# liyi14/mx-DeepIM

Measured on NVIDIA B200. Metric: 480x640 4-iter pose refinements/sec, higher is better.
Workload: dtype fp16

## Files before the change

### mx-deepim_b200/csrc/conv_igemm.cuh

```cuda
#pragma once
#include <cuda.h>
#include <cuda_fp16.h>
#include "common.cuh"

namespace dim {

struct ConvKParams {
  CUtensorMap a_map[4];
  CUtensorMap a_lo_map[4];
  CUtensorMap b_map;
  CUtensorMap b_lo_map;
  CUtensorMap b2_map;
  CUtensorMap b2_lo_map;
  int KH, KW, stride, cchunks;
  int BW, BH, n_col_tiles;
  int Hq, Ho, Wo, Bn;
  int out_Hp, out_Wp, out_py, out_px, Cout;
  int kblocks, ksplit;
  int f16;
  uint32_t idesc;
  float slope;
  const float *bias;
  __nv_bfloat16 *out_hi, *out_lo;
  float *partial;
  int in_off_r, in_off_c;
  int out_sy, out_sx, out_oy, out_ox, out_H, out_W, out_cs, out_coff;
  struct PixBuf { const __nv_bfloat16 *p; int Hp, Wp, py, px, cs, coff; } addend, mask;
  int mask_climit;
};

namespace ptx {

__device__ __forceinline__ uint32_t smem_u32(const void *p) { return (uint32_t)__cvta_generic_to_shared(p); }

__device__ __forceinline__ bool elect_one() {
  uint32_t pred;
  asm volatile(
      "{\n\t.reg .pred p;\n\telect.sync _|p, 0xFFFFFFFF;\n\tselp.u32 %0, 1, 0, p;\n\t}"
      : "=r"(pred));
  return pred != 0;
}

// ... 128 lines not shown
  d |= (uint64_t)((saddr & 0x3FFFFu) >> 4);
  d |= (uint64_t)1 << 16;
  d |= (uint64_t)((sbo_bytes >> 4) & 0x3FFFu) << 32;
  d |= (uint64_t)1 << 46;
  d |= (uint64_t)layout_type << 61;
  return d;
}

}

__device__ __forceinline__ void sts128(uint32_t addr, uint4 v) {
  asm volatile("st.shared.v4.b32 [%0], {%1, %2, %3, %4};" ::"r"(addr), "r"(v.x), "r"(v.y), "r"(v.z), "r"(v.w) : "memory");
}
__device__ __forceinline__ uint4 lds128(uint32_t addr) {
  uint4 v;
  asm volatile("ld.shared.v4.b32 {%0, %1, %2, %3}, [%4];" : "=r"(v.x), "=r"(v.y), "=r"(v.z), "=r"(v.w) : "r"(addr) : "memory");
  return v;
}
__device__ __forceinline__ float4 lds128f(uint32_t addr) {
  float4 v;
  asm volatile("ld.shared.v4.f32 {%0, %1, %2, %3}, [%4];" : "=f"(v.x), "=f"(v.y), "=f"(v.z), "=f"(v.w) : "r"(addr));
  return v;
}

__device__ __forceinline__ uint32_t pack2_f16(float a, float b) {
  uint32_t r;
  asm("cvt.rn.satfinite.f16x2.f32 %0, %1, %2;" : "=r"(r) : "f"(b), "f"(a));
  return r;
}
__device__ __forceinline__ uint32_t pack2_bf16(float a, float b) {
  uint32_t r;
  asm("cvt.rn.bf16x2.f32 %0, %1, %2;" : "=r"(r) : "f"(b), "f"(a));
  return r;
}

template <bool SPLIT3>
__device__ __forceinline__ void epilogue_store64(const uint32_t *r, const float *bias_s, float slope, uint8_t *stage,
                                                 __nv_bfloat16 *out_hi, __nv_bfloat16 *out_lo, long long my_off,
                                                 bool my_valid, int lane, bool f16 = false) {
  __align__(16) uint32_t h[32];
  __align__(16) uint32_t l[SPLIT3 ? 32 : 4];
  const uint32_t ba = ptx::smem_u32(bias_s), sa = ptx::smem_u32(stage);
#pragma unroll
  for (int j = 0; j < 64; j += 4) {
    const float4 b4 = lds128f(ba + j * 4);
    float v0 = __uint_as_float(r[j]) + b4.x, v1 = __uint_as_float(r[j + 1]) + b4.y;
    float v2 = __uint_as_float(r[j + 2]) + b4.z, v3 = __uint_as_float(r[j + 3]) + b4.w;
    v0 = v0 > 0.f ? v0 : v0 * slope;
    v1 = v1 > 0.f ? v1 : v1 * slope;
    v2 = v2 > 0.f ? v2 : v2 * slope;
    v3 = v3 > 0.f ? v3 : v3 * slope;
    if (!SPLIT3 && f16) {
      h[j >> 1] = pack2_f16(v0, v1);
      h[(j >> 1) + 1] = pack2_f16(v2, v3);
    } else {
      const uint32_t h0 = pack2_bf16(v0, v1), h1 = pack2_bf16(v2, v3);
      h[j >> 1] = h0;
      h[(j >> 1) + 1] = h1;
      if (SPLIT3) {
        l[j >> 1] = pack2_bf16(v0 - __uint_as_float(h0 << 16), v1 - __uint_as_float(h0 & 0xFFFF0000u));
        l[(j >> 1) + 1] = pack2_bf16(v2 - __uint_as_float(h1 << 16), v3 - __uint_as_float(h1 & 0xFFFF0000u));
      }
    }
  }
  const unsigned vmask = __ballot_sync(0xffffffffu, my_valid);
  const int ch = lane & 7;
#pragma unroll
  for (int pass = 0; pass < (SPLIT3 ? 2 : 1); ++pass) {
    const uint32_t *src = pass ? l : h;
    __nv_bfloat16 *out = pass ? out_lo : out_hi;
#pragma unroll
    for (int c = 0; c < 8; ++c)
      sts128(sa + lane * 128 + ((c ^ (lane & 7)) << 4), *reinterpret_cast<const uint4 *>(src + c * 4));
    __syncwarp();
#pragma unroll
    for (int i = 0; i < 8; ++i) {
      const int row = i * 4 + (lane >> 3);
      const long long off = __shfl_sync(0xffffffffu, my_off, row);
      const uint4 v = lds128(sa + row * 128 + ((ch ^ (row & 7)) << 4));
      if ((vmask >> row) & 1u) *reinterpret_cast<uint4 *>(out + off + ch * 8) = v;
    }
    __syncwarp();
  }
}

template <bool SPLIT3, bool LINEAR = false, bool BIAS_REG = false>
__device__ __forceinline__ void epilogue_store32(const uint32_t *r, const float *bias_s, float slope, uint8_t *stage,
                                                 __nv_bfloat16 *out_hi, __nv_bfloat16 *out_lo, long long my_off,
                                                 bool my_valid, int lane, bool f16, int n_valid = 32, int row_stride = 0) {
  __align__(16) uint32_t h[16];
  __align__(16) uint32_t l[SPLIT3 ? 16 : 4];
  const uint32_t ba = BIAS_REG ? 0u : ptx::smem_u32(bias_s), sa = ptx::smem_u32(stage);
#pragma unroll
  for (int j = 0; j < 32; j += 4) {
    const float4 b4 = BIAS_REG ? make_float4(bias_s[j], bias_s[j + 1], bias_s[j + 2], bias_s[j + 3]) : lds128f(ba + j * 4);
    float v0 = __uint_as_float(r[j]) + b4.x, v1 = __uint_as_float(r[j + 1]) + b4.y;
    float v2 = __uint_as_float(r[j + 2]) + b4.z, v3 = __uint_as_float(r[j + 3]) + b4.w;
    v0 = v0 > 0.f ? v0 : v0 * slope;
    v1 = v1 > 0.f ? v1 : v1 * slope;
    v2 = v2 > 0.f ? v2 : v2 * slope;
    v3 = v3 > 0.f ? v3 : v3 * slope;
    if (!SPLIT3 && f16) {
      h[j >> 1] = pack2_f16(v0, v1);
      h[(j >> 1) + 1] = pack2_f16(v2, v3);
    } else {
      const uint32_t h0 = pack2_bf16(v0, v1), h1 = pack2_bf16(v2, v3);
      h[j >> 1] = h0;
      h[(j >> 1) + 1] = h1;
      if (SPLIT3) {
        l[j >> 1] = pack2_bf16(v0 - __uint_as_float(h0 << 16), v1 - __uint_as_float(h0 & 0xFFFF0000u));
        l[(j >> 1) + 1] = pack2_bf16(v2 - __uint_as_float(h1 << 16), v3 - __uint_as_float(h1 & 0xFFFF0000u));
      }
    }
  }
  const unsigned vmask = LINEAR ? 0u : __ballot_sync(0xffffffffu, my_valid);
  const int ch = lane & 3;
#pragma unroll
  for (int pass = 0; pass < (SPLIT3 ? 2 : 1); ++pass) {
    const uint32_t *src = pass ? l : h;
    __nv_bfloat16 *out = pass ? out_lo : out_hi;
#pragma unroll
    for (int c = 0; c < 4; ++c)
      sts128(sa + lane * 64 + ((c ^ ((lane >> 1) & 3)) << 4), *reinterpret_cast<const uint4 *>(src + c * 4));
    __syncwarp();
#pragma unroll
    for (int i = 0; i < 4; ++i) {
      const int row = i * 8 + (lane >> 2);
      const uint4 v = lds128(sa + row * 64 + ((ch ^ ((row >> 1) & 3)) << 4));
      if (LINEAR) {
        if (row < n_valid) *reinterpret_cast<uint4 *>(out + my_off + (long long)row * row_stride + ch * 8) = v;
      } else {
        const long long off = __shfl_sync(0xffffffffu, my_off, row);
        if ((vmask >> row) & 1u) *reinterpret_cast<uint4 *>(out + off + ch * 8) = v;
      }
    }
    __syncwarp();
  }
// ... 42 lines not shown
    const int row = i * 4 + (lane >> 3);
    const long long off = __shfl_sync(0xffffffffu, my_off, row);
    const uint4 v = lds128(sa + row * 128 + ((ch ^ (row & 7)) << 4));
    if ((vmask >> row) & 1u) *reinterpret_cast<uint4 *>(p.out_hi + off + ch * 8) = v;
  }
  __syncwarp();
}

template <int BLOCK_N, int BLOCK_K, int STAGES, bool SPLIT3, bool RESIDENT_B, int KBLOCKS_RES>
struct ConvSmem2 {
  static constexpr int A_BYTES = 128 * BLOCK_K * 2;
  static constexpr int B_BYTES = BLOCK_N * BLOCK_K * 2;
  static constexpr int NPREC = SPLIT3 ? 2 : 1;
  static constexpr int STAGE_BYTES = (A_BYTES + (RESIDENT_B ? 0 : B_BYTES)) * NPREC;
  static constexpr int RES_BYTES = RESIDENT_B ? KBLOCKS_RES * B_BYTES * NPREC : 0;
  static constexpr int EPI_BYTES = 4 * 4096 + 4096 ;
  static constexpr int TOTAL = STAGES * STAGE_BYTES + RES_BYTES + EPI_BYTES + 1024  + 512 ;
};

__device__ __forceinline__ void mbar_arrive(uint64_t *bar) {
  asm volatile("mbarrier.arrive.shared::cta.b64 _, [%0];" ::"r"(ptx::smem_u32(bar)) : "memory");
}

template <int BLOCK_N, int BLOCK_K, int STAGES, bool SPLIT3, bool RESIDENT_B, int KBLOCKS_RES, int EPI = 0>
__global__ void __launch_bounds__(192) conv_igemm_persistent_kernel(const __grid_constant__ ConvKParams p,
                                                                    const int total_tiles, const int n_tiles) {
  using S = ConvSmem2<BLOCK_N, BLOCK_K, STAGES, SPLIT3, RESIDENT_B, KBLOCKS_RES>;
  constexpr uint32_t LAYOUT = (BLOCK_K == 64) ? 2u : 4u;
  constexpr uint32_t SBO = 8u * BLOCK_K * 2u;
  constexpr uint32_t ACC_COLS = BLOCK_N < 32 ? 32 : BLOCK_N;
  constexpr uint32_t TMEM_COLS = 2 * ACC_COLS;

  extern __shared__ uint8_t smem_raw[];
  uint8_t *smem = reinterpret_cast<uint8_t *>((reinterpret_cast<uintptr_t>(smem_raw) + 1023) & ~(uintptr_t)1023);
  uint8_t *res = smem + STAGES * S::STAGE_BYTES;
  uint8_t *epi = res + S::RES_BYTES;
  float *bias_s = reinterpret_cast<float *>(epi + 4 * 4096);
  uint64_t *full_bar = reinterpret_cast<uint64_t *>(epi + S::EPI_BYTES);
  uint64_t *empty_bar = full_bar + STAGES;
  uint64_t *tmem_full_bar = empty_bar + STAGES;
  uint64_t *tmem_empty_bar = tmem_full_bar + 2;
  uint64_t *res_bar = tmem_empty_bar + 2;
  uint32_t *tmem_slot = reinterpret_cast<uint32_t *>(res_bar + 1);

  const int warp = threadIdx.x >> 5, lane = threadIdx.x & 31;
  const int kb0 = 0, kb1 = p.kblocks;

  if (warp == 0 && lane == 0) {
    for (int s = 0; s < STAGES; ++s) {
      ptx::mbar_init(&full_bar[s], 1);
      ptx::mbar_init(&empty_bar[s], 1);
    }
    for (int a = 0; a < 2; ++a) {
      ptx::mbar_init(&tmem_full_bar[a], 1);
      ptx::mbar_init(&tmem_empty_bar[a], 4);
    }
    ptx::mbar_init(res_bar, 1);
    ptx::fence_barrier_init();
    ptx::prefetch_tmap(&p.b_map);
    ptx::prefetch_tmap(&p.a_map[0]);
  }
  for (int c = threadIdx.x; c < p.Cout && c < 1024; c += blockDim.x) bias_s[c] = p.bias ? p.bias[c] : 0.f;
  if (warp == 1) ptx::tmem_alloc(tmem_slot, TMEM_COLS);
  ptx::tc_fence_before();
  __syncthreads();
  ptx::tc_fence_after();
  const uint32_t tmem_base = *tmem_slot;

  if (warp == 0) {
    {
      if (RESIDENT_B) {
        ptx::mbar_expect_tx(res_bar, (uint32_t)S::RES_BYTES);
        for (int kb = 0; kb < KBLOCKS_RES; ++kb) {
          ptx::tma_load_2d(res + kb * S::B_BYTES, &p.b_map, res_bar, kb * BLOCK_K, 0);
          if (SPLIT3) ptx::tma_load_2d(res + (KBLOCKS_RES + kb) * S::B_BYTES, &p.b_lo_map, res_bar, kb * BLOCK_K, 0);
        }
      }
      const uint32_t tx = (uint32_t)(p.BW * p.BH * BLOCK_K * 2 + (RESIDENT_B ? 0 : BLOCK_N * BLOCK_K * 2)) * S::NPREC;
      int s = 0;
      uint32_t ph = 0;
      for (int tile = blockIdx.x; tile < total_tiles; tile += gridDim.x) {
        const int nt = tile % n_tiles, mt = tile / n_tiles;
        const int col_tile = mt % p.n_col_tiles, row_tile = mt / p.n_col_tiles;
        const int g0 = row_tile * p.BH, ow0 = col_tile * p.BW, n0 = nt * BLOCK_N;
        for (int kb = kb0; kb < kb1; ++kb) {
          ptx::mbar_wait(&empty_bar[s], ph ^ 1u);
          const int tap = kb / p.cchunks, cc = kb - tap * p.cchunks;
          const int kh = tap / p.KW, kw = tap - kh * p.KW;
          int view = 0, dr = kh, dc = kw;
          if (p.stride == 2) {
            view = ((kh & 1) << 1) | (kw & 1);
            dr = kh >> 1;
            dc = kw >> 1;
          }
          uint8_t *st = smem + s * S::STAGE_BYTES;
          if (EPI) { dr += p.in_off_r; dc += p.in_off_c; }
          if (ptx::elect_one()) {
            ptx::mbar_expect_tx_raw(&full_bar[s], tx);
            ptx::tma_load_3d_raw(st, &p.a_map[view], &full_bar[s], cc * BLOCK_K, ow0 + dc, g0 + dr);
            uint8_t *nxt = st + S::A_BYTES;
            if (!RESIDENT_B) {
              ptx::tma_load_2d_raw(nxt, &p.b_map, &full_bar[s], kb * BLOCK_K, n0);
              nxt += S::B_BYTES;
            }
            if (SPLIT3) {
              ptx::tma_load_3d_raw(nxt, &p.a_lo_map[view], &full_bar[s], cc * BLOCK_K, ow0 + dc, g0 + dr);
              if (!RESIDENT_B) ptx::tma_load_2d_raw(nxt + S::A_BYTES, &p.b_lo_map, &full_bar[s], kb * BLOCK_K, n0);
            }
          }
          __syncwarp();
          if (++s == STAGES) { s = 0; ph ^= 1u; }
        }
      }
    }
  } else if (warp == 1) {
    {
      if (RESIDENT_B) {
        ptx::mbar_wait(res_bar, 0);
        ptx::tc_fence_after();
      }
      int s = 0, as = 0;
      uint32_t ph = 0, aph = 0;
      for (int tile = blockIdx.x; tile < total_tiles; tile += gridDim.x) {
        ptx::mbar_wait(&tmem_empty_bar[as], aph ^ 1u);
        ptx::tc_fence_after();
        const uint32_t tmem_acc = tmem_base + (uint32_t)as * ACC_COLS;
        for (int kb = kb0; kb < kb1; ++kb) {
          ptx::mbar_wait(&full_bar[s], ph);
          ptx::tc_fence_after();
          const uint32_t a_hi = ptx::smem_u32(smem + s * S::STAGE_BYTES);
          uint32_t b_hi, a_lo, b_lo;
          if (RESIDENT_B) {
            b_hi = ptx::smem_u32(res + kb * S::B_BYTES);
            b_lo = ptx::smem_u32(res + (KBLOCKS_RES + kb) * S::B_BYTES);
            a_lo = a_hi + S::A_BYTES;
          } else {
            b_hi = a_hi + S::A_BYTES;
            a_lo = b_hi + S::B_BYTES;
            b_lo = a_lo + S::A_BYTES;
          }
          if (ptx::elect_one()) {
            const uint64_t da0 = ptx::umma_desc(a_hi, SBO, LAYOUT), db0 = ptx::umma_desc(b_hi, SBO, LAYOUT);
            const uint64_t dal0 = ptx::umma_desc(a_lo, SBO, LAYOUT), dbl0 = ptx::umma_desc(b_lo, SBO, LAYOUT);
#pragma unroll
            for (int k = 0; k < BLOCK_K / 16; ++k) {
              const uint32_t acc = (kb > kb0 || k > 0) ? 1u : 0u;
              const uint64_t da = da0 + (uint64_t)(2 * k), db = db0 + (uint64_t)(2 * k);
              ptx::umma_f16_raw(tmem_acc, da, db, p.idesc, acc);
              if (SPLIT3) {
                ptx::umma_f16_raw(tmem_acc, dal0 + (uint64_t)(2 * k), db, p.idesc, 1u);
                ptx::umma_f16_raw(tmem_acc, da, dbl0 + (uint64_t)(2 * k), p.idesc, 1u);
              }
            }
            ptx::umma_commit_raw(&empty_bar[s]);
          }
          __syncwarp();
          if (++s == STAGES) { s = 0; ph ^= 1u; }
        }
        ptx::umma_commit(&tmem_full_bar[as]);
        if (++as == 2) { as = 0; aph ^= 1u; }
      }
    }
  } else {
    const int quad = warp & 3;
    const int m = quad * 32 + lane;
    const int bh = m / p.BW, bw = m - bh * p.BW;
    uint8_t *stg = epi + (warp - 2) * 4096;
    int as = 0;
    uint32_t aph = 0;
    for (int tile = blockIdx.x; tile < total_tiles; tile += gridDim.x) {
      ptx::mbar_wait(&tmem_full_bar[as], aph);
      ptx::tc_fence_after();
      const uint32_t trow = tmem_base + ((uint32_t)(quad * 32) << 16) + (uint32_t)as * ACC_COLS;
      if (EPI == 1) {
        const int nt = tile % n_tiles, mt = tile / n_tiles;
        const int col_tile = mt % p.n_col_tiles, row_tile = mt / p.n_col_tiles;
        const int g = row_tile * p.BH + bh, ow = col_tile * p.BW + bw, n0 = nt * BLOCK_N;
        const int n_img = g / p.Hq, oh = g - n_img * p.Hq;
        const int y = oh * p.out_sy + p.out_oy, x = ow * p.out_sx + p.out_ox;
        const bool valid = (m < p.BW * p.BH) && (n_img < p.Bn) && (oh < p.Ho) && (ow < p.Wo) && y >= 0 && y < p.out_H &&
                           x >= 0 && x < p.out_W;
        const long long my_off =
            (((long long)n_img * p.out_Hp + y + p.out_py) * p.out_Wp + x + p.out_px) * p.out_cs + p.out_coff + n0;
        const long long add_off =
            (((long long)n_img * p.addend.Hp + y + p.addend.py) * p.addend.Wp + x + p.addend.px) * p.addend.cs + p.addend.coff + n0;
        const long long mask_off =
            (((long long)n_img * p.mask.Hp + y + p.mask.py) * p.mask.Wp + x + p.mask.px) * p.mask.cs + p.mask.coff + n0;
#pragma unroll 1
        for (int c = 0; c < BLOCK_N; c += 64) {
          uint32_t r[64];
          ptx::tmem_ld_32x32(trow + c, r);
          ptx::tmem_ld_32x32(trow + c + 32, r + 32);
          if (c + 64 >= BLOCK_N) {
            ptx::tc_fence_before();
            __syncwarp();
            if (lane == 0) mbar_arrive(&tmem_empty_bar[as]);
          }
          epilogue_generic64(r, p, bias_s + ((n0 + c) & 1023), stg, my_off + c, add_off + c, mask_off + c, valid,
                             n0 + c < p.mask_climit, n0 + c < p.Cout, lane);
        }
      } else {
        const int nt = tile % n_tiles, mt = tile / n_tiles;
        const int col_tile = mt % p.n_col_tiles, row_tile = mt / p.n_col_tiles;
        const int g = row_tile * p.BH + bh, ow = col_tile * p.BW + bw, n0 = nt * BLOCK_N;
        const int n_img = g / p.Hq, oh = g - n_img * p.Hq;
        const bool valid = (m < p.BW * p.BH) && (n_img < p.Bn) && (oh < p.Ho) && (ow < p.Wo);
        const long long my_off =
            (((long long)n_img * p.out_Hp + oh + p.out_py) * p.out_Wp + ow + p.out_px) * p.Cout + n0;
#pragma unroll 1
        for (int c = 0; c < BLOCK_N; c += 64) {
          uint32_t r[64];
          ptx::tmem_ld_32x32(trow + c, r);
          ptx::tmem_ld_32x32(trow + c + 32, r + 32);
          if (c + 64 >= BLOCK_N) {
            ptx::tc_fence_before();
            __syncwarp();
            if (lane == 0) mbar_arrive(&tmem_empty_bar[as]);
          }
          epilogue_store64<SPLIT3>(r, bias_s + n0 + c, p.slope, stg, p.out_hi, p.out_lo, my_off + c, valid, lane, p.f16 != 0);
        }
      }
      if (++as == 2) { as = 0; aph ^= 1u; }
    }
  }
  ptx::tc_fence_before();
  __syncthreads();
  if (warp == 1) {
    ptx::tc_fence_after();
    ptx::tmem_dealloc(tmem_base, TMEM_COLS);
  }
}

__device__ __forceinline__ void tma_load_4d(void *dst, const CUtensorMap *map, uint64_t *bar, int c0, int c1, int c2,
                                            int c3) {
  if (ptx::elect_one())
  asm volatile(
      "cp.async.bulk.tensor.4d.shared::cluster.global.mbarrier::complete_tx::bytes [%0], [%1, {%3, %4, %5, %6}], [%2];" ::
          "r"(ptx::smem_u32(dst)),
      "l"((uint64_t)map), "r"(ptx::smem_u32(bar)), "r"(c0), "r"(c1), "r"(c2), "r"(c3)
      : "memory");
}
__device__ __forceinline__ uint64_t umma_desc_interleave(uint32_t saddr, uint32_t lbo_bytes, uint32_t sbo_bytes) {
// ... 137 lines not shown
    const int quad = warp & 3, set = (warp - 2) >> 2;
    uint8_t *stg = epi + (warp - 2) * STG;
    const int as = set;
    uint32_t aph = 0;
    const int n_cols_valid = min(p.BW, p.Wo - ow0) - quad * 32;
    for (int t = set; t < n_rows; t += 2) {
      const int g = g_lo + t;
      const int n_img = g / p.Hq, oh = g - n_img * p.Hq;
      const bool row_ok = (n_img < p.Bn) && (oh < p.Ho);
      ptx::mbar_wait(&tmem_full_bar[as], aph);
      ptx::tc_fence_after();
      const uint32_t trow = tmem_base + ((uint32_t)(quad * 32) << 16) + (uint32_t)as * ACC_COLS;
      const long long warp_off =
          (((long long)n_img * p.out_Hp + oh + p.out_py) * p.out_Wp + (ow0 + quad * 32) + p.out_px) * 64;
      uint32_t r[64];
      ptx::tmem_ld_32x32(trow, r);
      ptx::tmem_ld_32x32(trow + 32, r + 32);
      ptx::tc_fence_before();
      __syncwarp();
      if (lane == 0) mbar_arrive(&tmem_empty_bar[as]);
#pragma unroll
      for (int half = 0; half < 2; ++half)
        epilogue_store32<SPLIT3, true>(r + half * 32, bias_s + half * 32, p.slope, stg, p.out_hi, p.out_lo, warp_off + half * 32,
                                             true, lane, p.f16 != 0, row_ok ? n_cols_valid : 0, 64);
      aph ^= 1u;
    }
  }
  ptx::tc_fence_before();
  __syncthreads();
  if (warp == 1) {
    ptx::tc_fence_after();
    ptx::tmem_dealloc(tmem_base, TMEM_COLS);
  }
}

template <int STAGES>
__global__ void __launch_bounds__(320) conv1_stack_kernel(const __grid_constant__ ConvKParams p, const int rows_total,
                                                          const int rows_per_chunk, const int chunks_per_col,
                                                          const int strip_bytes ) {
  constexpr uint32_t TMEM_COLS = 512;
  constexpr int B_BYTES = 64 * 32 * 2 , DW_BYTES = 4 * B_BYTES, RES_BYTES = 4 * DW_BYTES;
  constexpr int EPI_BYTES = 8 * 2048 + 256;
  extern __shared__ uint8_t smem_raw[];
  uint8_t *smem = reinterpret_cast<uint8_t *>((reinterpret_cast<uintptr_t>(smem_raw) + 511) & ~(uintptr_t)511);
  uint8_t *res = smem;
  uint8_t *ring = smem + RES_BYTES;
  uint8_t *epi = ring + STAGES * strip_bytes;
// ... 123 lines not shown
      const bool mine = v >= 3;
      int n_img = 0, oh = 0;
      if (mine) { n_img = g / p.Hq; oh = g - n_img * p.Hq; }
      const bool row_ok = mine && (n_img < p.Bn) && (oh < p.Ho);
      ptx::mbar_wait(&acc_full_bar[v & 7], ((uint32_t)(v >> 3)) & 1u);
      ptx::tc_fence_after();
      const uint32_t tcol = tmem_base + ((uint32_t)(quad * 32) << 16) + (uint32_t)((v & 7) * 64);
      uint32_t r[64];
      if (row_ok) {
        ptx::tmem_ld_32x32(tcol, r);
        ptx::tmem_ld_32x32(tcol + 32, r + 32);
      }
      ptx::tmem_zero_32x32(tcol);
      ptx::tmem_zero_32x32(tcol + 32);
      ptx::tc_fence_before();
      __syncwarp();
      if (lane == 0) mbar_arrive(&acc_empty_bar[v & 7]);
      if (row_ok) {
        const long long warp_off =
            (((long long)n_img * p.out_Hp + oh + p.out_py) * p.out_Wp + (ow0 + quad * 32) + p.out_px) * 64;
#pragma unroll
        for (int half = 0; half < 2; ++half)
          epilogue_store32<false, true, true>(r + half * 32, breg + half * 32, p.slope, stg, p.out_hi, p.out_lo, warp_off + half * 32,
                                              true, lane, p.f16 != 0, n_cols_valid, 64);
      }
    }
  }
  ptx::tc_fence_before();
  __syncthreads();
  if (warp == 1) {
    ptx::tc_fence_after();
    ptx::tmem_dealloc(tmem_base, TMEM_COLS);
  }
}

namespace ptx2 {
__device__ __forceinline__ uint32_t cluster_ctarank() {
  uint32_t r;
  asm volatile("mov.u32 %0, %%cluster_ctarank;" : "=r"(r));
  return r;
}
__device__ __forceinline__ void cluster_sync() {
  asm volatile("barrier.cluster.arrive.release.aligned;\n\tbarrier.cluster.wait.acquire.aligned;" ::: "memory");
}
constexpr uint32_t kPeerBitMask = 0xFEFFFFFFu;
__device__ __forceinline__ void tma_load_3d(void *dst, const CUtensorMap *map, uint64_t *bar, int c0, int c1, int c2) {
  if (ptx::elect_one())
// ... 203 lines not shown
          ptx::tmem_ld_32x32(trow + c, r);
          if (valid) {
#pragma unroll
            for (int j = 0; j < 32; j += 4)
              *reinterpret_cast<uint4 *>(dst + c + j) = make_uint4(r[j], r[j + 1], r[j + 2], r[j + 3]);
          }
        }
        ptx::tc_fence_before();
        __syncwarp();
        if (lane == 0) ptx2::mbar_arrive_leader(&tmem_empty_bar[as]);
      } else {
        const long long my_off =
            (((long long)n_img * p.out_Hp + oh + p.out_py) * p.out_Wp + ow + p.out_px) * p.Cout + n0;
#pragma unroll 1
        for (int c = 0; c < BLOCK_N; c += 64) {
          uint32_t r[64];
          ptx::tmem_ld_32x32(trow + c, r);
          ptx::tmem_ld_32x32(trow + c + 32, r + 32);
          if (c + 64 >= BLOCK_N) {
            ptx::tc_fence_before();
            __syncwarp();
            if (lane == 0) ptx2::mbar_arrive_leader(&tmem_empty_bar[as]);
          }
          epilogue_store64<SPLIT3>(r, bias_s + n0 + c, p.slope, stg, p.out_hi, p.out_lo, my_off + c, valid, lane, p.f16 != 0);
        }
      }
      if (++as == 2) { as = 0; aph ^= 1u; }
    }
  }
  ptx::tc_fence_before();
  __syncthreads();
  ptx2::cluster_sync();
  if (warp == 1) {
    ptx::tc_fence_after();
    ptx2::tmem_dealloc(tmem_base, TMEM_COLS);
  }
}

static __global__ void __launch_bounds__(256) conv_splitk_finalize_kernel(const float *partial, int ksplit, int npix,
                                                                   int Cout, int Ho, int Wo, int out_Hp, int out_Wp,
                                                                   int out_py, int out_px, const float *bias,
                                                                   float slope, __nv_bfloat16 *out_hi,
                                                                   __nv_bfloat16 *out_lo, int f16) {
  const size_t idx4 = ((size_t)blockIdx.x * blockDim.x + threadIdx.x) * 4;
  if (idx4 >= (size_t)npix * Cout) return;
  const size_t opix = idx4 / Cout;
  const int c = (int)(idx4 - opix * Cout);
// ... 26 lines not shown
```

### mx-deepim_b200/csrc/net.cu

```cuda
#include <cuda_fp16.h>
#include <string.h>

#include <mutex>

#include "net_state.cuh"

namespace dim {

static void build_geometry(NetState *ns, int H, int W) {
  int h = H, w = W;
  for (int i = 0; i < 10; ++i) {
    const LayerSpec &s = kLayers[i];
    LayerGeom &g = ns->g[i];
    g.Cin = s.Cin; g.Cout = s.Cout; g.k = s.k; g.stride = s.stride; g.pad = s.pad;
    g.Hin = h; g.Win = w;
    g.Ho = (h + 2 * s.pad - s.k) / s.stride + 1;
    g.Wo = (w + 2 * s.pad - s.k) / s.stride + 1;
    if (g.Ho < 1) g.Ho = 1;
    if (g.Wo < 1) g.Wo = 1;
    int Hp = h + 2 * s.pad, Wp = w + 2 * s.pad;
    if (s.stride == 2) { Hp += Hp & 1; Wp += Wp & 1; }
    g.py = g.px = s.pad;
    if (i == 0) {
      g.rows = Hp / 2; g.cols = Wp / 2; g.Cbuf = 32;
// ... 131 lines not shown
      const uint64_t str[1] = {Ktot * 2};
      const uint32_t box[2] = {(uint32_t)g.BLOCK_K, (uint32_t)g.BLOCK_N};
      __nv_bfloat16 *wop = f16 ? ns->w_f16[i] : ns->w_hi[i];
      if (int rc = encode_map(&kp.b_map, wop, 2, dims, str, box, g.BLOCK_K)) return rc;
      if (int rc = encode_map(&kp.b_lo_map, ns->w_lo[i], 2, dims, str, box, g.BLOCK_K)) return rc;
      const uint32_t box2[2] = {(uint32_t)g.BLOCK_K, (uint32_t)(g.BLOCK_N / 2)};
      if (int rc = encode_map(&kp.b2_map, wop, 2, dims, str, box2, g.BLOCK_K)) return rc;
      if (int rc = encode_map(&kp.b2_lo_map, ns->w_lo[i], 2, dims, str, box2, g.BLOCK_K)) return rc;
    }
    kp.KH = g.KH; kp.KW = g.KW; kp.stride = g.stride_eff; kp.cchunks = g.Ceff / g.BLOCK_K;
    kp.BW = g.BW; kp.BH = g.BH; kp.n_col_tiles = g.n_col_tiles;
    kp.Hq = g.Hq; kp.Ho = g.Ho; kp.Wo = g.Wo; kp.Bn = B;
    if (i < 9) {
      const LayerGeom &nx = ns->g[i + 1];
      kp.out_Hp = nx.rows; kp.out_Wp = nx.cols; kp.out_py = nx.py; kp.out_px = nx.px;
    } else {
      kp.out_Hp = g.Ho; kp.out_Wp = g.Wo; kp.out_py = 0; kp.out_px = 0;
    }
    kp.Cout = g.Cout;
    kp.kblocks = g.kblocks;
    kp.ksplit = tm.ksplit[i] = choose_ksplit(ns, g, B);
    kp.idesc = make_idesc(g.pair ? 256 : 128, g.BLOCK_N, f16);
    kp.f16 = f16 ? 1 : 0;
    kp.slope = 0.1f;
    kp.bias = ns->bias[i];
    kp.out_hi = ns->act_hi[i + 1];
    kp.out_lo = ns->act_lo[i + 1];
    kp.partial = ns->conv_partial;
  }
  return 0;
}

template <bool F16>
__device__ __forceinline__ void mma_bf16_16816(float *c, const uint32_t *a, uint32_t b0, uint32_t b1) {
  if (F16)
    asm volatile(
        "mma.sync.aligned.m16n8k16.row.col.f32.f16.f16.f32 {%0,%1,%2,%3}, {%4,%5,%6,%7}, {%8,%9}, {%0,%1,%2,%3};"
        : "+f"(c[0]), "+f"(c[1]), "+f"(c[2]), "+f"(c[3])
        : "r"(a[0]), "r"(a[1]), "r"(a[2]), "r"(a[3]), "r"(b0), "r"(b1));
  else
    asm volatile(
        "mma.sync.aligned.m16n8k16.row.col.f32.bf16.bf16.f32 {%0,%1,%2,%3}, {%4,%5,%6,%7}, {%8,%9}, {%0,%1,%2,%3};"
        : "+f"(c[0]), "+f"(c[1]), "+f"(c[2]), "+f"(c[3])
        : "r"(a[0]), "r"(a[1]), "r"(a[2]), "r"(a[3]), "r"(b0), "r"(b1));
}

// ... 258 lines not shown
    for (int o = 0; o < 256; ++o)
      for (int c = 0; c < 1024; ++c)
        for (int hw = 0; hw < 80; ++hw) p[(size_t)o * FC6_K + (size_t)hw * 1024 + c] = W[10][(size_t)o * FC6_K + (size_t)c * 80 + hw];
    std::vector<__nv_bfloat16> hb, lb, fb;
    split_bf16(p.data(), p.size(), hb, lb, fb);
    if (int rc = upload(ctx, &ns->fc6_w_hi, hb)) return rc;
    if (int rc = upload(ctx, &ns->fc6_w_lo, lb)) return rc;
    if (int rc = upload(ctx, &ns->fc6_w_f16, fb)) return rc;
    if (int rc = upload(ctx, &ns->fc6_b, std::vector<float>(Bv[10], Bv[10] + 256))) return rc;
    std::vector<float> t((size_t)256 * 256);
    for (int o = 0; o < 256; ++o)
      for (int k = 0; k < 256; ++k) t[(size_t)k * 256 + o] = W[11][(size_t)o * 256 + k];
    if (int rc = upload(ctx, &ns->fc7_wT, t)) return rc;
    if (int rc = upload(ctx, &ns->fc7_b, std::vector<float>(Bv[11], Bv[11] + 256))) return rc;
    if (int rc = upload(ctx, &ns->rot_w, std::vector<float>(W[12], W[12] + 4 * 256))) return rc;
    if (int rc = upload(ctx, &ns->rot_b, std::vector<float>(Bv[12], Bv[12] + 4))) return rc;
    if (int rc = upload(ctx, &ns->trans_w, std::vector<float>(W[13], W[13] + 3 * 256))) return rc;
    if (int rc = upload(ctx, &ns->trans_b, std::vector<float>(Bv[13], Bv[13] + 3))) return rc;
  }
  ns->loaded = true;
  return 0;
}

template <int BN, int BK, int ST, bool S3, bool RES, int KRES>
static int launch_conv2(NetState *ns, const ConvKParams &kp, int total_tiles, int n_tiles, int cap, cudaStream_t st) {
  using S = ConvSmem2<BN, BK, ST, S3, RES, KRES>;
  static bool attr_set = false;
  if (!attr_set) {
    DIM_CHECK(cudaFuncSetAttribute(conv_igemm_persistent_kernel<BN, BK, ST, S3, RES, KRES>,
                                   cudaFuncAttributeMaxDynamicSharedMemorySize, S::TOTAL));
    attr_set = true;
  }
  const int grid = total_tiles < cap ? total_tiles : cap;
  conv_igemm_persistent_kernel<BN, BK, ST, S3, RES, KRES><<<grid, 192, S::TOTAL, st>>>(kp, total_tiles, n_tiles);
  DIM_LAUNCH_CHECK();
  return 0;
}

template <int BN, int ST, bool S3>
static int launch_pair(const ConvKParams &kp, int pair_tiles, int n_tiles, int sms, cudaStream_t st) {
  using S = ConvSmemPair<BN, ST, S3>;
  static bool attr_set = false;
  if (!attr_set) {
    DIM_CHECK(cudaFuncSetAttribute(conv_igemm_pair_kernel<BN, ST, S3>, cudaFuncAttributeMaxDynamicSharedMemorySize,
                                   S::TOTAL));
    attr_set = true;
  }
  const int pairs = pair_tiles < sms / 2 ? pair_tiles : sms / 2;
  conv_igemm_pair_kernel<BN, ST, S3><<<2 * pairs, 192, S::TOTAL, st>>>(kp, pair_tiles, n_tiles);
  DIM_LAUNCH_CHECK();
  return 0;
}

void net_input_geometry(dim_ctx *ctx, int *rows, int *cols, int *pad, __nv_bfloat16 **hi, __nv_bfloat16 **lo) {
  NetState *ns = ctx->net;
  *rows = ns->g[0].rows; *cols = ns->g[0].cols; *pad = ns->g[0].py;
  *hi = ns->act_hi[0]; *lo = ns->act_lo[0];
// ... 7 lines not shown
  DIM_REQUIRE(precision == DIM_PREC_BF16 || precision == DIM_PREC_BF16X3 || precision == DIM_PREC_FP16,
              "unknown precision (DIM_PREC_BF16 / DIM_PREC_BF16X3 / DIM_PREC_FP16)");
  const bool s3 = precision == DIM_PREC_BF16X3, f16 = precision == DIM_PREC_FP16;
  const int key = B + (f16 ? kF16MapKey : 0);
  auto it = ns->maps.find(key);
  if (it == ns->maps.end()) {
    TensorMaps tm;
    if (int rc = build_maps(ns, B, f16, tm)) return rc;
    it = ns->maps.emplace(key, tm).first;
  }
  const TensorMaps &tm = it->second;
  if (ns->repack_done) DIM_CHECK(cudaStreamWaitEvent(st, ns->repack_done, 0));
  if (s3 && ns->lo_stale)
    if (int rc = train_refresh_lo(ctx, st)) return rc;
  if (f16 && ns->f16_stale)
    if (int rc = net_refresh_f16(ctx, st)) return rc;
  if (ns->layer_events) DIM_CHECK(cudaEventRecord(ns->layer_events[0], st));
  for (int i = 0; i < 10; ++i) {
    const LayerGeom &g = tm.g[i];
    const ConvKParams &kp = tm.kp[i];
    const int n_tiles = g.Cout / g.BLOCK_N;
    const int total_tiles = cdiv(B * g.Hq, g.BH) * g.n_col_tiles * n_tiles * kp.ksplit;
    const int sms = ns->num_sms;
    int rc;
    if (i == 0) {
      const int rows_total = B * g.Hq;
      int chunks = sms / g.n_col_tiles;
      if (chunks > cdiv(rows_total, 16)) chunks = cdiv(rows_total, 16);
      if (chunks < 1) chunks = 1;
      const int rpc = cdiv(rows_total, chunks);
      chunks = cdiv(rows_total, rpc);
      const int strip_bytes = cdiv((g.BW + 3) * 64, 128) * 128;
      const int grid = g.n_col_tiles * chunks;
      if (s3) {
        constexpr int ST = 5;
        const int smem_bytes = 2 * 16 * 4096 + ST * 2 * strip_bytes + (8 * 2048 + 256) + 1024 + 512;
        DIM_REQUIRE(smem_bytes <= 227 * 1024, "conv1 (bf16x3): image too wide for the rolling-strip ring");
        static int set1 = 0;
        if (set1 < smem_bytes) { DIM_CHECK(cudaFuncSetAttribute(conv1_roll_kernel<ST, true>, cudaFuncAttributeMaxDynamicSharedMemorySize, smem_bytes)); set1 = smem_bytes; }
        conv1_roll_kernel<ST, true><<<grid, 320, smem_bytes, st>>>(kp, rows_total, rpc, chunks, strip_bytes);
      } else if (ns->conv1_stack) {
        constexpr int ST = 6;
        const int smem_bytes = 16 * 4096 + ST * strip_bytes + (8 * 2048 + 256) + 512 + 512;
        static int set3 = 0;
        if (set3 < smem_bytes) { DIM_CHECK(cudaFuncSetAttribute(conv1_stack_kernel<ST>, cudaFuncAttributeMaxDynamicSharedMemorySize, smem_bytes)); set3 = smem_bytes; }
        conv1_stack_kernel<ST><<<grid, 320, smem_bytes, st>>>(kp, rows_total, rpc, chunks, strip_bytes);
      } else {
        constexpr int ST = 8;
        const int smem_bytes = 16 * 4096 + ST * strip_bytes + (8 * 2048 + 256) + 1024 + 512;
        static int set0 = 0;
        if (set0 < smem_bytes) { DIM_CHECK(cudaFuncSetAttribute(conv1_roll_kernel<ST, false>, cudaFuncAttributeMaxDynamicSharedMemorySize, smem_bytes)); set0 = smem_bytes; }
        conv1_roll_kernel<ST, false><<<grid, 320, smem_bytes, st>>>(kp, rows_total, rpc, chunks, strip_bytes);
      }
      DIM_LAUNCH_CHECK();
      rc = 0;
    }
    else if (g.pair) {
      const int m_tiles = cdiv(B * g.Hq, g.BH) * g.n_col_tiles;
      const int pair_tiles = cdiv(m_tiles, 2) * n_tiles * kp.ksplit;
      if (g.BLOCK_N == 128 && g.pair == 2 && !s3)
        rc = launch_pair<128, 3, false>(kp, pair_tiles, n_tiles, 2 * sms, st);
      else if (g.BLOCK_N == 128)
        rc = s3 ? launch_pair<128, 4, true>(kp, pair_tiles, n_tiles, sms, st) : launch_pair<128, 8, false>(kp, pair_tiles, n_tiles, sms, st);
      else
        rc = s3 ? launch_pair<256, 3, true>(kp, pair_tiles, n_tiles, sms, st) : launch_pair<256, 6, false>(kp, pair_tiles, n_tiles, sms, st);
    } else if (g.BLOCK_N <= 128) {
      rc = s3 ? launch_conv2<128, 64, 3, true, false, 0>(ns, kp, total_tiles, n_tiles, sms, st)
              : (g.occ == 2 ? launch_conv2<128, 64, 2, false, false, 0>(ns, kp, total_tiles, n_tiles, 2 * sms, st)
                            : launch_conv2<128, 64, 5, false, false, 0>(ns, kp, total_tiles, n_tiles, sms, st));
    }
    else
      rc = s3 ? launch_conv2<256, 64, 2, true, false, 0>(ns, kp, total_tiles, n_tiles, sms, st)
              : launch_conv2<256, 64, 4, false, false, 0>(ns, kp, total_tiles, n_tiles, sms, st);
    if (rc) return rc;
    if (ns->layer_events && i < 9) DIM_CHECK(cudaEventRecord(ns->layer_events[i + 1], st));
    if (kp.ksplit > 1) {
      const int npix = B * g.Ho * g.Wo;
      const size_t n4 = (size_t)npix * g.Cout / 4;
      conv_splitk_finalize_kernel<<<(unsigned)cdiv((int)n4, 256), 256, 0, st>>>(
          ns->conv_partial, kp.ksplit, npix, g.Cout, g.Ho, g.Wo, kp.out_Hp, kp.out_Wp, kp.out_py, kp.out_px,
          ns->bias[i], 0.1f, ns->act_hi[i + 1], s3 ? ns->act_lo[i + 1] : nullptr, f16 ? 1 : 0);
      DIM_LAUNCH_CHECK();
    }
  }
  if (ns->layer_events) DIM_CHECK(cudaEventRecord(ns->layer_events[10], st));
  if (after_conv) DIM_CHECK(cudaEventRecord(after_conv, st));
  if (s3)
    fc6_mma_kernel<true><<<FC6_SPLITS, 256, 0, st>>>(ns->act_hi[10], ns->act_lo[10], ns->fc6_w_hi, ns->fc6_w_lo, B,
                                                     ctx->max_batch, ns->fc6_partial);
  else if (f16)
    fc6_mma_kernel<false, true><<<FC6_SPLITS, 256, 0, st>>>(ns->act_hi[10], nullptr, ns->fc6_w_f16, nullptr, B,
                                                            ctx->max_batch, ns->fc6_partial);
  else
    fc6_mma_kernel<false><<<FC6_SPLITS, 256, 0, st>>>(ns->act_hi[10], nullptr, ns->fc6_w_hi, nullptr, B,
                                                      ctx->max_batch, ns->fc6_partial);
  DIM_LAUNCH_CHECK();
  head_kernel<<<B, 1024, 0, st>>>(ns->fc6_partial, ctx->max_batch, ns->fc6_b, ns->fc7_wT, ns->fc7_b, ns->rot_w,
                                 ns->rot_b, ns->trans_w, ns->trans_b, zoom_factor, rot_out, trans_out, se3_out, ns->save_h6,
                                 ns->save_h7);
  DIM_LAUNCH_CHECK();
  return 0;
}

bool net_graph_safe(dim_ctx *ctx) {
  NetState *ns = ctx->net;
  return ns && ns->loaded && !ns->layer_events && !ns->train_aliased;
}

int net_set_option(dim_ctx *ctx, const char *key, int value) {
  NetState *ns = ctx->net;
  DIM_REQUIRE(ns != nullptr, "net not created");
  if (!strcmp(key, "pair_mask")) ns->pair_mask = value & 0x3FE;
  else if (!strcmp(key, "conv1_stack")) ns->conv1_stack = value != 0;
  else { set_error("dim_debug_set_option: unknown key '%s'", key); return 2; }
  DIM_CHECK(cudaDeviceSynchronize());
  ns->maps.clear();
  return 0;
}

int net_layer_profile(dim_ctx *ctx, int enable, float *ms10) {
  NetState *ns = ctx->net;
  DIM_REQUIRE(ns != nullptr, "net not created");
  if (enable && !ns->layer_events) {
    ns->layer_events = new cudaEvent_t[11];
    for (int i = 0; i < 11; ++i) DIM_CHECK(cudaEventCreate(&ns->layer_events[i]));
  }
  if (ms10 && ns->layer_events) {
    DIM_CHECK(cudaDeviceSynchronize());
    for (int i = 0; i < 10; ++i) DIM_CHECK(cudaEventElapsedTime(&ms10[i], ns->layer_events[i], ns->layer_events[i + 1]));
  }
  if (!enable && ns->layer_events) {
    for (int i = 0; i < 11; ++i) cudaEventDestroy(ns->layer_events[i]);
    delete[] ns->layer_events;
    ns->layer_events = nullptr;
  }
  return 0;
// ... 25 lines not shown
```

### mx-deepim_b200/csrc/net_state.cuh

```cuda
#pragma once
#include <map>

#include "conv_igemm.cuh"

namespace dim {

struct LayerSpec {
  const char *name;
  int Cout, Cin, k, stride, pad;
};
static const LayerSpec kLayers[10] = {
    {"flow_conv1", 64, 8, 7, 2, 3},  {"conv2", 128, 64, 5, 2, 2},   {"conv3", 256, 128, 5, 2, 2},
    {"conv3_1", 256, 256, 3, 1, 1},  {"conv4", 512, 256, 3, 2, 1},  {"conv4_1", 512, 512, 3, 1, 1},
    {"conv5", 512, 512, 3, 2, 1},    {"conv5_1", 512, 512, 3, 1, 1}, {"conv6", 1024, 512, 3, 2, 1},
    {"conv6_1", 1024, 1024, 3, 1, 1}};

struct LayerGeom {
  int Cin, Cout, k, stride, pad, Hin, Win, Ho, Wo;
  int rows, cols, Cbuf, py, px;
  int KH, KW, stride_eff, Ceff, Hq;
  int BLOCK_N, BLOCK_K, BW, BH, n_col_tiles, kblocks;
  int pair;
  int occ;
};
// ... 4 lines not shown
  LayerGeom g[10];
};

__host__ __device__ inline int conv1_kslot(int dw, int ph, int pw) { return dw == 3 ? pw * 16 + ph * 8 : ph * 16 + pw * 8; }

struct NetState {
  LayerGeom g[10];
  __nv_bfloat16 *w_hi[10] = {}, *w_lo[10] = {};
  __nv_bfloat16 *w_f16[10] = {};
  float *bias[10] = {};
  __nv_bfloat16 *act_hi[11] = {}, *act_lo[11] = {};
  size_t act_elems_per_image[11] = {};
  __nv_bfloat16 *fc6_w_hi = nullptr, *fc6_w_lo = nullptr;
  __nv_bfloat16 *fc6_w_f16 = nullptr;
  bool train_aliased = false;
  bool f16_stale = false;
  float *fc6_b = nullptr, *fc7_wT = nullptr, *fc7_b = nullptr, *rot_w = nullptr, *rot_b = nullptr,
        *trans_w = nullptr, *trans_b = nullptr;
  float *fc6_partial = nullptr;
  float *conv_partial = nullptr;
  size_t conv_partial_elems = 0;
  bool conv1_stack = true;
  int pair_mask = 1 << 1;
  cudaEvent_t *layer_events = nullptr;
  bool loaded = false, net_ok = false;
  float *save_h6 = nullptr, *save_h7 = nullptr;
  cudaEvent_t repack_done = nullptr;
  bool lo_stale = false;
  std::map<int, TensorMaps> maps;
  int max_batch = 0, num_sms = 148;
};

static constexpr int FC6_K = 1024 * 8 * 10;
static constexpr int FC6_KC = 256;
static constexpr int FC6_SPLITS = FC6_K / FC6_KC;


int encode_map(CUtensorMap *m, void *base, int rank, const uint64_t *dims, const uint64_t *strides_bytes,
               const uint32_t *box, int block_k );
uint32_t make_idesc(int M, int N, bool f16 = false);
static constexpr int kF16MapKey = 1 << 20;
int train_refresh_lo(dim_ctx *ctx, cudaStream_t st);
int net_forward(dim_ctx *ctx, int B, int precision, const float *zoom_factor, float *rot_out, float *trans_out,
                float *se3_out, cudaStream_t st, cudaEvent_t after_conv);

template <typename T>
// ... 11 lines not shown
```

Before: 5761.

## Add Cout-major conv tiles and direct 256-bit global epilogue stores

Adds a Cout-major variant of the persistent implicit-GEMM conv kernel for layers with BLOCK_N 128. Each tile runs a 128x256 MMA with weights as the M operand and two pixel tiles as N, then transposes the accumulators in-warp with shuffles so each lane writes a pixel's channels. Separately, the epilogues can now write straight from registers with st.global.v8 instead of staging through shared memory, and both paths are on by default through new debug options. This cuts shared-memory staging and improves MMA shape use, but the 32x32 shuffle transpose is costly, the Cout-major path skips the split-k finalize, and the per-lane direct stores are strided rather than coalesced.

```diff
diff --git a/mx-deepim_b200/csrc/conv_igemm.cuh b/mx-deepim_b200/csrc/conv_igemm.cuh
--- a/mx-deepim_b200/csrc/conv_igemm.cuh
+++ b/mx-deepim_b200/csrc/conv_igemm.cuh
@@ -18,6 +18,7 @@
   int out_Hp, out_Wp, out_py, out_px, Cout;
   int kblocks, ksplit;
   int f16;
+  int direct_store;
   uint32_t idesc;
   float slope;
   const float *bias;
@@ -192,6 +193,11 @@
   asm volatile("ld.shared.v4.f32 {%0, %1, %2, %3}, [%4];" : "=f"(v.x), "=f"(v.y), "=f"(v.z), "=f"(v.w) : "r"(addr));
   return v;
 }
+__device__ __forceinline__ void stg256(void *p, const uint32_t *v) {
+  asm volatile("st.global.v8.b32 [%0], {%1, %2, %3, %4, %5, %6, %7, %8};" ::"l"(p), "r"(v[0]), "r"(v[1]), "r"(v[2]),
+               "r"(v[3]), "r"(v[4]), "r"(v[5]), "r"(v[6]), "r"(v[7])
+               : "memory");
+}
 
 __device__ __forceinline__ uint32_t pack2_f16(float a, float b) {
   uint32_t r;
@@ -207,7 +213,7 @@
 template <bool SPLIT3>
 __device__ __forceinline__ void epilogue_store64(const uint32_t *r, const float *bias_s, float slope, uint8_t *stage,
                                                  __nv_bfloat16 *out_hi, __nv_bfloat16 *out_lo, long long my_off,
-                                                 bool my_valid, int lane, bool f16 = false) {
+                                                 bool my_valid, int lane, bool f16, bool direct) {
   __align__(16) uint32_t h[32];
   __align__(16) uint32_t l[SPLIT3 ? 32 : 4];
   const uint32_t ba = ptx::smem_u32(bias_s), sa = ptx::smem_u32(stage);
@@ -233,6 +239,17 @@
       }
     }
   }
+  if (direct) {
+    if (my_valid) {
+#pragma unroll
+      for (int pass = 0; pass < (SPLIT3 ? 2 : 1); ++pass) {
+        __nv_bfloat16 *out = (pass ? out_lo : out_hi) + my_off;
+#pragma unroll
+        for (int c = 0; c < 4; ++c) stg256(out + c * 16, (pass ? l : h) + c * 8);
+      }
+    }
+    return;
+  }
   const unsigned vmask = __ballot_sync(0xffffffffu, my_valid);
   const int ch = lane & 7;
 #pragma unroll
@@ -257,7 +274,8 @@
 template <bool SPLIT3, bool LINEAR = false, bool BIAS_REG = false>
 __device__ __forceinline__ void epilogue_store32(const uint32_t *r, const float *bias_s, float slope, uint8_t *stage,
                                                  __nv_bfloat16 *out_hi, __nv_bfloat16 *out_lo, long long my_off,
-                                                 bool my_valid, int lane, bool f16, int n_valid = 32, int row_stride = 0) {
+                                                 bool my_valid, int lane, bool f16, bool direct, int n_valid = 32,
+                                                 int row_stride = 0) {
   __align__(16) uint32_t h[16];
   __align__(16) uint32_t l[SPLIT3 ? 16 : 4];
   const uint32_t ba = BIAS_REG ? 0u : ptx::smem_u32(bias_s), sa = ptx::smem_u32(stage);
@@ -283,6 +301,18 @@
       }
     }
   }
+  if (direct) {
+    const long long off = LINEAR ? my_off + (long long)lane * row_stride : my_off;
+    if (LINEAR ? lane < n_valid : my_valid) {
+#pragma unroll
+      for (int pass = 0; pass < (SPLIT3 ? 2 : 1); ++pass) {
+        __nv_bfloat16 *out = (pass ? out_lo : out_hi) + off;
+        stg256(out, pass ? l : h);
+        stg256(out + 16, (pass ? l : h) + 8);
+      }
+    }
+    return;
+  }
   const unsigned vmask = LINEAR ? 0u : __ballot_sync(0xffffffffu, my_valid);
   const int ch = lane & 3;
 #pragma unroll
@@ -371,9 +401,26 @@
   asm volatile("mbarrier.arrive.shared::cta.b64 _, [%0];" ::"r"(ptx::smem_u32(bar)) : "memory");
 }
 
-template <int BLOCK_N, int BLOCK_K, int STAGES, bool SPLIT3, bool RESIDENT_B, int KBLOCKS_RES, int EPI = 0>
+__device__ __forceinline__ void warp_transpose32(float *v, int lane) {
+#pragma unroll
+  for (int s = 16; s > 0; s >>= 1) {
+    const bool up = (lane & s) != 0;
+#pragma unroll
+    for (int i = 0; i < 32; ++i) {
+      if (i & s) continue;
+      const float x = __shfl_xor_sync(0xffffffffu, up ? v[i] : v[i + s], s);
+      if (up) v[i] = x;
+      else v[i + s] = x;
+    }
+  }
+}
+
+template <int BLOCK_N, int BLOCK_K, int STAGES, bool SPLIT3, bool RESIDENT_B, int KBLOCKS_RES, int EPI = 0,
+          bool COUT_MAJOR = false>
 __global__ void __launch_bounds__(192) conv_igemm_persistent_kernel(const __grid_constant__ ConvKParams p,
                                                                     const int total_tiles, const int n_tiles) {
+  static_assert(!COUT_MAJOR || (BLOCK_N == 256 && BLOCK_K == 64 && !SPLIT3 && !RESIDENT_B && EPI == 0),
+                "Cout-major tiles: 128 x 256 single-pass MMAs with the plain epilogue");
   using S = ConvSmem2<BLOCK_N, BLOCK_K, STAGES, SPLIT3, RESIDENT_B, KBLOCKS_RES>;
   constexpr uint32_t LAYOUT = (BLOCK_K == 64) ? 2u : 4u;
   constexpr uint32_t SBO = 8u * BLOCK_K * 2u;
@@ -394,6 +441,7 @@
 
   const int warp = threadIdx.x >> 5, lane = threadIdx.x & 31;
   const int kb0 = 0, kb1 = p.kblocks;
+  const int m_tiles = COUT_MAJOR ? (p.Bn * p.Hq + p.BH - 1) / p.BH * p.n_col_tiles : 0;
 
   if (warp == 0 && lane == 0) {
     for (int s = 0; s < STAGES; ++s) {
@@ -425,13 +473,17 @@
           if (SPLIT3) ptx::tma_load_2d(res + (KBLOCKS_RES + kb) * S::B_BYTES, &p.b_lo_map, res_bar, kb * BLOCK_K, 0);
         }
       }
-      const uint32_t tx = (uint32_t)(p.BW * p.BH * BLOCK_K * 2 + (RESIDENT_B ? 0 : BLOCK_N * BLOCK_K * 2)) * S::NPREC;
+      const uint32_t tx = COUT_MAJOR ? (uint32_t)(128 * BLOCK_K * 2 + 2 * p.BW * p.BH * BLOCK_K * 2)
+                                     : (uint32_t)(p.BW * p.BH * BLOCK_K * 2 + (RESIDENT_B ? 0 : BLOCK_N * BLOCK_K * 2)) * S::NPREC;
       int s = 0;
       uint32_t ph = 0;
       for (int tile = blockIdx.x; tile < total_tiles; tile += gridDim.x) {
-        const int nt = tile % n_tiles, mt = tile / n_tiles;
+        const int nt = tile % n_tiles;
+        const int mt = COUT_MAJOR ? 2 * (tile / n_tiles) : tile / n_tiles;
+        const int mt1 = COUT_MAJOR ? min(mt + 1, m_tiles - 1) : 0;
         const int col_tile = mt % p.n_col_tiles, row_tile = mt / p.n_col_tiles;
-        const int g0 = row_tile * p.BH, ow0 = col_tile * p.BW, n0 = nt * BLOCK_N;
+        const int g0 = row_tile * p.BH, ow0 = col_tile * p.BW, n0 = nt * (COUT_MAJOR ? 128 : BLOCK_N);
+        const int g1 = mt1 / p.n_col_tiles * p.BH, ow1 = mt1 % p.n_col_tiles * p.BW;
         for (int kb = kb0; kb < kb1; ++kb) {
           ptx::mbar_wait(&empty_bar[s], ph ^ 1u);
           const int tap = kb / p.cchunks, cc = kb - tap * p.cchunks;
@@ -444,7 +496,15 @@
           }
           uint8_t *st = smem + s * S::STAGE_BYTES;
           if (EPI) { dr += p.in_off_r; dc += p.in_off_c; }
-          if (ptx::elect_one()) {
+          if (COUT_MAJOR) {
+            if (ptx::elect_one()) {
+              ptx::mbar_expect_tx_raw(&full_bar[s], tx);
+              ptx::tma_load_2d_raw(st, &p.b_map, &full_bar[s], kb * BLOCK_K, n0);
+              ptx::tma_load_3d_raw(st + S::A_BYTES, &p.a_map[view], &full_bar[s], cc * BLOCK_K, ow0 + dc, g0 + dr);
+              ptx::tma_load_3d_raw(st + S::A_BYTES + 128 * BLOCK_K * 2, &p.a_map[view], &full_bar[s], cc * BLOCK_K, ow1 + dc,
+                                   g1 + dr);
+            }
+          } else if (ptx::elect_one()) {
             ptx::mbar_expect_tx_raw(&full_bar[s], tx);
             ptx::tma_load_3d_raw(st, &p.a_map[view], &full_bar[s], cc * BLOCK_K, ow0 + dc, g0 + dr);
             uint8_t *nxt = st + S::A_BYTES;
@@ -468,6 +528,7 @@
         ptx::mbar_wait(res_bar, 0);
         ptx::tc_fence_after();
       }
+      const uint32_t idesc = COUT_MAJOR ? (p.idesc & 0x1FFFFu) | ((uint32_t)(BLOCK_N >> 3) << 17) | (8u << 24) : p.idesc;
       int s = 0, as = 0;
       uint32_t ph = 0, aph = 0;
       for (int tile = blockIdx.x; tile < total_tiles; tile += gridDim.x) {
@@ -495,10 +556,10 @@
             for (int k = 0; k < BLOCK_K / 16; ++k) {
               const uint32_t acc = (kb > kb0 || k > 0) ? 1u : 0u;
               const uint64_t da = da0 + (uint64_t)(2 * k), db = db0 + (uint64_t)(2 * k);
-              ptx::umma_f16_raw(tmem_acc, da, db, p.idesc, acc);
+              ptx::umma_f16_raw(tmem_acc, da, db, idesc, acc);
               if (SPLIT3) {
-                ptx::umma_f16_raw(tmem_acc, dal0 + (uint64_t)(2 * k), db, p.idesc, 1u);
-                ptx::umma_f16_raw(tmem_acc, da, dbl0 + (uint64_t)(2 * k), p.idesc, 1u);
+                ptx::umma_f16_raw(tmem_acc, dal0 + (uint64_t)(2 * k), db, idesc, 1u);
+                ptx::umma_f16_raw(tmem_acc, da, dbl0 + (uint64_t)(2 * k), idesc, 1u);
               }
             }
             ptx::umma_commit_raw(&empty_bar[s]);
@@ -521,7 +582,41 @@
       ptx::mbar_wait(&tmem_full_bar[as], aph);
       ptx::tc_fence_after();
       const uint32_t trow = tmem_base + ((uint32_t)(quad * 32) << 16) + (uint32_t)as * ACC_COLS;
-      if (EPI == 1) {
+      if (COUT_MAJOR) {
+        const int mp = tile / n_tiles, co = (tile % n_tiles) * 128 + quad * 32;
+        const float b = bias_s[co + lane];
+        const bool f16 = p.f16 != 0;
+#pragma unroll 1
+        for (int c = 0; c < BLOCK_N; c += 32) {
+          uint32_t r[32];
+          ptx::tmem_ld_32x32(trow + c, r);
+          if (c + 32 >= BLOCK_N) {
+            ptx::tc_fence_before();
+            __syncwarp();
+            if (lane == 0) mbar_arrive(&tmem_empty_bar[as]);
+          }
+          float v[32];
+#pragma unroll
+          for (int j = 0; j < 32; ++j) {
+            const float x = __uint_as_float(r[j]) + b;
+            v[j] = x > 0.f ? x : x * p.slope;
+          }
+          warp_transpose32(v, lane);
+          const int j = c + lane, mt = 2 * mp + (j >> 7), mm = j & 127;
+          const int bh = mm / p.BW, bw = mm - bh * p.BW;
+          const int g = mt / p.n_col_tiles * p.BH + bh, ow = mt % p.n_col_tiles * p.BW + bw;
+          const int n_img = g / p.Hq, oh = g - n_img * p.Hq;
+          if (mt < m_tiles && mm < p.BW * p.BH && n_img < p.Bn && oh < p.Ho && ow < p.Wo) {
+            __align__(16) uint32_t h[16];
+#pragma unroll
+            for (int q = 0; q < 16; ++q) h[q] = f16 ? pack2_f16(v[2 * q], v[2 * q + 1]) : pack2_bf16(v[2 * q], v[2 * q + 1]);
+            __nv_bfloat16 *out =
+                p.out_hi + (((long long)n_img * p.out_Hp + oh + p.out_py) * p.out_Wp + ow + p.out_px) * p.Cout + co;
+            stg256(out, h);
+            stg256(out + 16, h + 8);
+          }
+        }
+      } else if (EPI == 1) {
         const int nt = tile % n_tiles, mt = tile / n_tiles;
         const int col_tile = mt % p.n_col_tiles, row_tile = mt / p.n_col_tiles;
         const int g = row_tile * p.BH + bh, ow = col_tile * p.BW + bw, n0 = nt * BLOCK_N;
@@ -566,7 +661,8 @@
             __syncwarp();
             if (lane == 0) mbar_arrive(&tmem_empty_bar[as]);
           }
-          epilogue_store64<SPLIT3>(r, bias_s + n0 + c, p.slope, stg, p.out_hi, p.out_lo, my_off + c, valid, lane, p.f16 != 0);
+          epilogue_store64<SPLIT3>(r, bias_s + n0 + c, p.slope, stg, p.out_hi, p.out_lo, my_off + c, valid, lane, p.f16 != 0,
+                                   p.direct_store != 0);
         }
       }
       if (++as == 2) { as = 0; aph ^= 1u; }
@@ -750,7 +846,7 @@
 #pragma unroll
       for (int half = 0; half < 2; ++half)
         epilogue_store32<SPLIT3, true>(r + half * 32, bias_s + half * 32, p.slope, stg, p.out_hi, p.out_lo, warp_off + half * 32,
-                                             true, lane, p.f16 != 0, row_ok ? n_cols_valid : 0, 64);
+                                             true, lane, p.f16 != 0, p.direct_store != 0, row_ok ? n_cols_valid : 0, 64);
       aph ^= 1u;
     }
   }
@@ -920,7 +1016,7 @@
 #pragma unroll
         for (int half = 0; half < 2; ++half)
           epilogue_store32<false, true, true>(r + half * 32, breg + half * 32, p.slope, stg, p.out_hi, p.out_lo, warp_off + half * 32,
-                                              true, lane, p.f16 != 0, n_cols_valid, 64);
+                                              true, lane, p.f16 != 0, p.direct_store != 0, n_cols_valid, 64);
       }
     }
   }
@@ -1170,7 +1266,8 @@
             __syncwarp();
             if (lane == 0) ptx2::mbar_arrive_leader(&tmem_empty_bar[as]);
           }
-          epilogue_store64<SPLIT3>(r, bias_s + n0 + c, p.slope, stg, p.out_hi, p.out_lo, my_off + c, valid, lane, p.f16 != 0);
+          epilogue_store64<SPLIT3>(r, bias_s + n0 + c, p.slope, stg, p.out_hi, p.out_lo, my_off + c, valid, lane, p.f16 != 0,
+                                   p.direct_store != 0);
         }
       }
       if (++as == 2) { as = 0; aph ^= 1u; }
diff --git a/mx-deepim_b200/csrc/net.cu b/mx-deepim_b200/csrc/net.cu
--- a/mx-deepim_b200/csrc/net.cu
+++ b/mx-deepim_b200/csrc/net.cu
@@ -177,6 +177,7 @@
     kp.ksplit = tm.ksplit[i] = choose_ksplit(ns, g, B);
     kp.idesc = make_idesc(g.pair ? 256 : 128, g.BLOCK_N, f16);
     kp.f16 = f16 ? 1 : 0;
+    kp.direct_store = (ns->direct_store >> i) & 1;
     kp.slope = 0.1f;
     kp.bias = ns->bias[i];
     kp.out_hi = ns->act_hi[i + 1];
@@ -481,17 +482,17 @@
   return 0;
 }
 
-template <int BN, int BK, int ST, bool S3, bool RES, int KRES>
+template <int BN, int BK, int ST, bool S3, bool RES, int KRES, bool CM = false>
 static int launch_conv2(NetState *ns, const ConvKParams &kp, int total_tiles, int n_tiles, int cap, cudaStream_t st) {
   using S = ConvSmem2<BN, BK, ST, S3, RES, KRES>;
   static bool attr_set = false;
   if (!attr_set) {
-    DIM_CHECK(cudaFuncSetAttribute(conv_igemm_persistent_kernel<BN, BK, ST, S3, RES, KRES>,
+    DIM_CHECK(cudaFuncSetAttribute(conv_igemm_persistent_kernel<BN, BK, ST, S3, RES, KRES, 0, CM>,
                                    cudaFuncAttributeMaxDynamicSharedMemorySize, S::TOTAL));
     attr_set = true;
   }
   const int grid = total_tiles < cap ? total_tiles : cap;
-  conv_igemm_persistent_kernel<BN, BK, ST, S3, RES, KRES><<<grid, 192, S::TOTAL, st>>>(kp, total_tiles, n_tiles);
+  conv_igemm_persistent_kernel<BN, BK, ST, S3, RES, KRES, 0, CM><<<grid, 192, S::TOTAL, st>>>(kp, total_tiles, n_tiles);
   DIM_LAUNCH_CHECK();
   return 0;
 }
@@ -545,6 +546,7 @@
     const int n_tiles = g.Cout / g.BLOCK_N;
     const int total_tiles = cdiv(B * g.Hq, g.BH) * g.n_col_tiles * n_tiles * kp.ksplit;
     const int sms = ns->num_sms;
+    const bool cout_major = i >= 1 && ns->conv2_cout_major && g.BLOCK_N == 128 && !s3;
     int rc;
     if (i == 0) {
       const int rows_total = B * g.Hq;
@@ -578,7 +580,10 @@
       DIM_LAUNCH_CHECK();
       rc = 0;
     }
-    else if (g.pair) {
+    else if (cout_major) {
+      const int m_tiles = cdiv(B * g.Hq, g.BH) * g.n_col_tiles;
+      rc = launch_conv2<256, 64, 4, false, false, 0, true>(ns, kp, cdiv(m_tiles, 2) * n_tiles, n_tiles, sms, st);
+    } else if (g.pair) {
       const int m_tiles = cdiv(B * g.Hq, g.BH) * g.n_col_tiles;
       const int pair_tiles = cdiv(m_tiles, 2) * n_tiles * kp.ksplit;
       if (g.BLOCK_N == 128 && g.pair == 2 && !s3)
@@ -597,7 +602,7 @@
               : launch_conv2<256, 64, 4, false, false, 0>(ns, kp, total_tiles, n_tiles, sms, st);
     if (rc) return rc;
     if (ns->layer_events && i < 9) DIM_CHECK(cudaEventRecord(ns->layer_events[i + 1], st));
-    if (kp.ksplit > 1) {
+    if (kp.ksplit > 1 && !cout_major) {
       const int npix = B * g.Ho * g.Wo;
       const size_t n4 = (size_t)npix * g.Cout / 4;
       conv_splitk_finalize_kernel<<<(unsigned)cdiv((int)n4, 256), 256, 0, st>>>(
@@ -635,6 +640,8 @@
   DIM_REQUIRE(ns != nullptr, "net not created");
   if (!strcmp(key, "pair_mask")) ns->pair_mask = value & 0x3FE;
   else if (!strcmp(key, "conv1_stack")) ns->conv1_stack = value != 0;
+  else if (!strcmp(key, "conv2_cout_major")) ns->conv2_cout_major = value != 0;
+  else if (!strcmp(key, "direct_store")) ns->direct_store = value & 0x3FF;
   else { set_error("dim_debug_set_option: unknown key '%s'", key); return 2; }
   DIM_CHECK(cudaDeviceSynchronize());
   ns->maps.clear();
diff --git a/mx-deepim_b200/csrc/net_state.cuh b/mx-deepim_b200/csrc/net_state.cuh
--- a/mx-deepim_b200/csrc/net_state.cuh
+++ b/mx-deepim_b200/csrc/net_state.cuh
@@ -50,6 +50,8 @@
   size_t conv_partial_elems = 0;
   bool conv1_stack = true;
   int pair_mask = 1 << 1;
+  bool conv2_cout_major = true;
+  int direct_store = 0x3FF;
   cudaEvent_t *layer_events = nullptr;
   bool loaded = false, net_ok = false;
   float *save_h6 = nullptr, *save_h7 = nullptr;
```

Result: faster. 5830, median of 6 (+1.2%).
